# marekrams/tnac4o

Hardware: AMD Instinct MI355X
Metric: PEPS-contraction ms/sweep, chimera L=2048 chi=64 (boundary-MPS sweep _setup_rhoT) (lower is better)
Workload: dtype f64; 1 GPU; chimera L=2048 (Nx=Ny=16, Nc=8), synthetic couplings seed 20260004, beta=3, chi=64; one sweep = 16 rows of MPO absorb + compress_mps; one step = the sweeps of the 4 lattice rotations of one instance; parallelism=1 GPU: 4 lattice rotations of one instance interleaved on 4 HIP streams, mode=sweep

## Files before the change

tnac4o_amd/csrc/common.h:

```cpp
#pragma once
#include <hip/hip_runtime.h>
#include <stdint.h>
#include <stdio.h>
#include <stdlib.h>
#include <string.h>

namespace tn {

void set_error(const char* fmt, ...);
const char* get_error();

inline int hip_fail(hipError_t e, const char* what) {
    set_error("%s: %s", what, hipGetErrorString(e));
    return (int)e > 0 ? (int)e : 1;
}

#define TN_CHECK_ARG(cond, msg)                \
    do {                                       \
        if (!(cond)) {                         \
            tn::set_error("%s: %s", __func__, msg); \
            return -1;                         \
        }                                      \
    } while (0)

// ... 78 lines not shown
struct Mat {
    double* p;
    int64_t rs, cs;
};
static inline Mat mat(double* p, int64_t rs, int64_t cs) { return Mat{p, rs, cs}; }
static inline Mat sub(Mat a, int64_t i, int64_t j) { return Mat{a.p + i * a.rs + j * a.cs, a.rs, a.cs}; }
static inline Mat tr(Mat a) { return Mat{a.p, a.cs, a.rs}; }

int gemm(hipStream_t st, int64_t M, int64_t N, int64_t K, double alpha, const double* A, int64_t rsa, int64_t csa,
         const double* B, int64_t rsb, int64_t csb, double beta, double* C, int64_t rsc, int64_t csc,
         int64_t batch = 1, int64_t bsa = 0, int64_t bsb = 0, int64_t bsc = 0, double* ws = nullptr,
         int64_t ws_bytes = 0);
int64_t gemm_ws_bytes(int64_t M, int64_t N, int64_t K, int64_t batch);
struct GemmExtra {
    const int* pairs = nullptr;
    const int* skip = nullptr;
    int pw = 0, mapA = 0, mapB = 0, mapC = 0;
    int force_splitk = 0;
    bool raw_partials = false;
    int* splitk_used = nullptr;
};
int gemm_forced_split(int64_t K, int s, int64_t* kchunk);
int gemm_ex(hipStream_t st, int64_t M, int64_t N, int64_t K, double alpha, const double* A, int64_t rsa, int64_t csa,
            const double* B, int64_t rsb, int64_t csb, double beta, double* C, int64_t rsc, int64_t csc, int64_t batch,
            int64_t bsa, int64_t bsb, int64_t bsc, double* ws, int64_t ws_bytes, const GemmExtra* x);

static inline int gemm(hipStream_t st, int64_t M, int64_t N, int64_t K, double alpha, Mat A, Mat B, double beta, Mat C,
                       double* ws = nullptr, int64_t ws_bytes = 0) {
    return gemm(st, M, N, K, alpha, A.p, A.rs, A.cs, B.p, B.rs, B.cs, beta, C.p, C.rs, C.cs, 1, 0, 0, 0, ws, ws_bytes);
}
int gemm_prof_family(int64_t M, int64_t N, int64_t K, int64_t rsc, int64_t csc);

int rank_update(hipStream_t st, int64_t m, int64_t n, int b, const double* W, int64_t wrs, int64_t wcs, const double* X, int64_t xrs,
                int64_t xcs, double* C, int64_t rsc, int64_t csc, const int* active);
static inline int rank_update(hipStream_t st, int64_t m, int64_t n, int b, Mat W, Mat X, Mat C, const int* active = nullptr) {
    return rank_update(st, m, n, b, W.p, W.rs, W.cs, X.p, X.rs, X.cs, C.p, C.rs, C.cs, active);
}

struct FactorProducts {
    int64_t Z, I, J, K1, N, Mhi, Mlo;
    const double* P; int64_t pz, pi, pk;
    const double* X; int64_t xk, xj, xn;
    const double* W; int64_t wm, wq;
    double* Out; int64_t oz, ohi, olo, on;
};
bool factor_products_fits(int64_t Z, int64_t I, int64_t J, int64_t K1, int64_t N, int64_t M);
inline bool factor_products_on() { return env_flag_on("TN_FACTOR_FUSED"); }
int factor_products(hipStream_t st, const FactorProducts& f);

constexpr int NBMAX = 64;

int gram_partial(hipStream_t st, const double* X, int64_t vs, int64_t es, int64_t L, int nvec, int w, const int* pairs,
                 int ngroups, int nchunk, double* part);
int gram_nchunk(int64_t L);

int eig_small(hipStream_t st, const double* part, int nchunk, int nvec, int ngroups, int mode, int max_sweeps,
              double dead_thresh, double* out, int* dead, int* nrot, double* maxoff, double relevant2 = 0.0, int allow_fast = 1);

int rows_times_small(hipStream_t st, double* X, int64_t rs, int64_t cs, int64_t nrows, int b, const double* S);

struct SvdRoundsJob {
    double* X; int64_t pitch, L; int nvp, w;
    const int* pairs; int ng, nr, nchunk;
    double* part; int64_t part_bytes; double* Js; int* nrot; double* maxoff;
    double relevant2, last_tol; int inner_first, inner_later;
    double* norms;
};
int svd_rounds_fused(hipStream_t st, const SvdRoundsJob& j);
int small_t_times_vecs(hipStream_t st, const double* S, double* X, int64_t vs, int64_t es, int64_t L, int nvec, int w,
// ... 143 lines not shown
```

tnac4o_amd/csrc/qr.hip:

```cpp
#include <stdlib.h>

#include <algorithm>
#include <map>
#include <mutex>
#include <tuple>
#include <vector>

#include "common.h"
#include "devprim.h"

namespace tn {

__global__ __launch_bounds__(256) void copy_mat_kernel(const double* __restrict__ S, int64_t srs, int64_t scs,
                                                       double* __restrict__ D, int64_t drs, int64_t dcs, int64_t m,
                                                       int64_t n, int colfast) {
    const int64_t e = (int64_t)blockIdx.x * 256 + threadIdx.x;
    if (e >= m * n) return;
    const int64_t i = colfast ? e / n : e % m, j = colfast ? e % n : e / m;
    D[i * drs + j * dcs] = S[i * srs + j * scs];
}

int copy_mat(hipStream_t st, const double* S, int64_t srs, int64_t scs, double* D, int64_t drs, int64_t dcs, int64_t m,
             int64_t n) {
    if (m <= 0 || n <= 0) return 0;
// ... 588 lines not shown
    for (int e = tid; e < k * n; e += 256) {
        const int i = e / n, c = e % n;
        const double sg = (As[i * n + i] < 0.0) ? -1.0 : 1.0;
        R[(int64_t)i * rrs + (int64_t)c * rcs] = (c >= i) ? sg * As[i * n + c] * ds : 0.0;
    }
    if (Q)
        for (int e = tid; e < m * k; e += 256) {
            const int r = e / k, j = e % k;
            const double sg = (As[j * n + j] < 0.0) ? -1.0 : 1.0;
            Q[(int64_t)r * qrs + (int64_t)j * qcs] = sg * Qs[e];
        }
}

static bool dbg_on() { static const bool on = env_flag_set("TN_DEBUG"); return on; }
static void dbg_check(hipStream_t st, const double* p, int64_t rs, int64_t cs, int64_t m, int64_t n, const char* what, int panel, int it) {
    if (!dbg_on()) return;
    std::vector<double> h((size_t)(m * n));
    (void)hipStreamSynchronize(st);
    for (int64_t i = 0; i < m; ++i)
        for (int64_t j = 0; j < n; ++j) (void)hipMemcpy(&h[i * n + j], p + i * rs + j * cs, 8, hipMemcpyDeviceToHost);
    double mx = 0, mn = 1e300; int bad = 0;
    for (double v : h) { if (!(v == v) || v > 1e300 || v < -1e300) ++bad; else { double a = v < 0 ? -v : v; if (a > mx) mx = a; if (a < mn) mn = a; } }
    fprintf(stderr, "[tn_qr dbg] panel %d it %d %-10s %lldx%lld nonfinite=%d max=%.3e min|.|=%.3e\n", panel, it, what, (long long)m, (long long)n, bad, mx, mn);
}

constexpr int QR_NBO_MAX = 256;
struct QrWs {
    double *Y, *Wq, *W, *UT, *UTq;
    double *G, *Tblk, *Zo, *Zo2, *tmpT;
    double *T, *X, *part, *Js, *Uinv, *Z, *Tri, *gemm_ws, *cn;
    int* dead;
    int* pairs;
    char* piv;
    int64_t gemm_ws_bytes;
    void* panel_ws;
    int64_t panel_bytes;
    void* cq_state = nullptr;
};

static int64_t qr_layout(int64_t m, int64_t n, int nb, char* base, QrWs* w) {
    const int64_t k = m < n ? m : n, P = cdiv(k, nb);
    WsCarve ws{base};
    double* Y = ws.take<double>(m * k * 8);
    double* Wq = ws.take<double>(m * k * 8);
    double* Wp = ws.take<double>(m * nb * 8);
    double* UT = ws.take<double>((int64_t)nb * nb * 8);
    double* UTq = ws.take<double>((int64_t)nb * nb * 8);
    double* T = ws.take<double>(P * nb * nb * 8);
    double* X = ws.take<double>((int64_t)nb * (n > k ? n : k) * 8);
    double* part = ws.take<double>((int64_t)64 * nb * nb * 8);
    double* Js = ws.take<double>((int64_t)nb * nb * 8);
    double* Uinv = ws.take<double>((int64_t)nb * nb * 8);
    double* Z = ws.take<double>(P * nb * nb * 8);
    double* Tri = ws.take<double>(P * nb * nb * 8);
    int* dead = ws.take<int>(nb * 4);
    double* cn = ws.take<double>(2 * n * 8);
    int* pairs = ws.take<int>((int64_t)2 * nb * 4);
    char* piv = ws.take<char>(1024 + n * 4);
    int64_t gw = (int64_t)64 * nb * (n > k ? n : k) * 8;
    {
        const int64_t tiles = cdiv(QR_NBO_MAX, 128) * cdiv(n > k ? n : k, 128);
        const int64_t g2 = (512 + 2 * tiles) * 128 * 128 * 8;
        if (g2 > gw) gw = g2;
    }
    double* gws = ws.take<double>(gw + 256);
    const int64_t nblk_o = cdiv(k, QR_NBO_MAX / 2);
    double* Gm = ws.take<double>((int64_t)QR_NBO_MAX * QR_NBO_MAX * 8);
    double* Tblk = ws.take<double>(nblk_o * QR_NBO_MAX * QR_NBO_MAX * 8);
    double* Zb = ws.take<double>((int64_t)QR_NBO_MAX * (n > k ? n : k) * 8);
    double* Zb2 = ws.take<double>((int64_t)QR_NBO_MAX * (n > k ? n : k) * 8);
    double* tmpT = ws.take<double>((int64_t)QR_NBO_MAX * 64 * 8);
    if (w) { w->G = Gm; w->Tblk = Tblk; w->Zo = Zb; w->Zo2 = Zb2; w->tmpT = tmpT; }
    const int64_t pb = cholqr_ws_bytes(m, nb < 32 ? nb : 32);
    void* pw = ws.take(pb);
    if (w) { w->panel_ws = pw; w->panel_bytes = pb; }
    if (w) { w->Wq = Wq; w->W = Wp; w->UT = UT; w->UTq = UTq; }
    if (w) { w->Y = Y; w->T = T; w->X = X; w->part = part; w->Js = Js; w->Uinv = Uinv; w->Z = Z; w->Tri = Tri;
             w->dead = dead; w->gemm_ws = gws; w->gemm_ws_bytes = gw; w->cn = cn; w->pairs = pairs; w->piv = piv; }
    return ws.total();
}

int64_t qr_ws_bytes(int64_t m, int64_t n, int nb) { return qr_layout(m, n, nb, nullptr, nullptr); }
struct QrCall {
    hipStream_t st;
    double* A; int64_t rs, cs, m, n; double* Q; int64_t qrs, qcs; double* R; int64_t rrs, rcs;
    int nb; void* ws; int64_t ws_bytes; double rank_tol;
    int64_t* keff_host; double* dropped2_host; int frob_exit; int64_t* pivot_perm_host; double* nf_out2; int* nf_done; bool* input_intact;
};
struct QrState {
    QrWs w;
    bool pivot, reveal, rowmajor, ru_on, wform;
    int64_t yrs, ycs, wrs, wcs;
    Mat Am, Ym, Wqm;
    int fbase = 0;
    double scale2 = -1.0;
};
struct QrPanel {
    int p, b; int64_t j0, mp;
    Mat Ap, Yp, Wp, Wqp;
    double* Tp;
};
static QrPanel panel_at(const QrCall& c, const QrState& s, int p, int64_t kend) {
    QrPanel pn;
    pn.p = p, pn.j0 = (int64_t)p * c.nb, pn.mp = c.m - pn.j0;
    pn.b = (int)((kend - pn.j0 < c.nb) ? kend - pn.j0 : c.nb);
    pn.Ap = sub(s.Am, pn.j0, pn.j0), pn.Yp = sub(s.Ym, pn.j0, pn.j0), pn.Wqp = sub(s.Wqm, pn.j0, pn.j0);
    pn.Wp = s.wform ? pn.Wqp : mat(s.w.W, s.wrs, s.wcs);
    pn.Tp = s.w.T + (int64_t)p * c.nb * c.nb;
    return pn;
}
#define QR_LAUNCH(c, kernel, grid, ...) \
// ... 155 lines not shown
        S->h.k_exit = j0 + b;
        S->h.stamp = p + 1;
        if (p == 0) { S->h.scale2 = fro2; S->h.dropped2 = 0.0; }
        S->h.active = 1;
        piv_post(mail, 1, j0 + b, stamp);
    }
}
__global__ __launch_bounds__(256) void swap_columns_dev_kernel(double* __restrict__ A, int64_t rs, int64_t cs, int64_t m, const PivState* __restrict__ S,
                                                               int* __restrict__ perm) {
    const int g = threadIdx.x >> 6;
    int src[16], dst[16];
#pragma unroll
    for (int i = 0; i < 16; ++i) { src[i] = S->src[g * 16 + i]; dst[i] = S->dst[g * 16 + i]; }
    const int active = S->h.active, ns = S->h.swap_n;
    if (active == 0 || ns <= 0 || ns > 64) return;
    if (blockIdx.x == gridDim.x - 1) {
        int old = 0;
        if ((int)threadIdx.x < ns) old = perm[S->src[threadIdx.x]];
        __syncthreads();
        if ((int)threadIdx.x < ns) perm[S->dst[threadIdx.x]] = old;
        return;
    }
    const int64_t r = (int64_t)blockIdx.x * 64 + (threadIdx.x & 63);
    const bool in = r < m;
    double* row = A + (in ? r : 0) * rs;
    double v[16];
#pragma unroll
    for (int i = 0; i < 16; ++i) { const int t = g * 16 + i; v[i] = (in && t < ns) ? row[(int64_t)src[i] * cs] : 0.0; }
    __syncthreads();
#pragma unroll
    for (int i = 0; i < 16; ++i) { const int t = g * 16 + i; if (in && t < ns) row[(int64_t)dst[i] * cs] = v[i]; }
}

constexpr int QMB = 128;
__global__ __launch_bounds__(256) void zero_above_panels_kernel(double* __restrict__ Y, int64_t rs, int64_t cs, int64_t k, int nb) {
    const int64_t J0 = (int64_t)blockIdx.y * QMB;
    const int bw = (int)((k - J0 < QMB) ? k - J0 : QMB);
    for (int e = blockIdx.x * 256 + threadIdx.x; e < bw * bw; e += gridDim.x * 256) {
        const int i = e / bw, j = e % bw;
        if (i / nb < j / nb) Y[(J0 + i) * rs + (J0 + j) * cs] = 0.0;
    }
}
__global__ __launch_bounds__(256) void apply_merged_T_kernel(const double* __restrict__ Z, int64_t nq, const double* __restrict__ G, int bw,
                                                             const double* __restrict__ T, int npan, double* __restrict__ X) {
    constexpr int NP = QMB / 32;
    __shared__ double xs[QMB][33];
    __shared__ double vs[32][33];
    __shared__ double gs[(NP - 1) * 32][QMB - 32 + 1];
    __shared__ double ts[NP][32][33];
    const int tid = threadIdx.x, lane = tid & 63, wave = tid >> 6;
    const int lr = lane & 15, lk = lane >> 4, ti = wave >> 1, tj = wave & 1;
    const int64_t c0 = (int64_t)blockIdx.x * 32;
    {
        double gv[12][3], tv[NP * 4];
#pragma unroll
        for (int u1 = 0; u1 < 12; ++u1)
#pragma unroll
            for (int u2 = 0; u2 < 3; ++u2) {
                const int i = (tid >> 5) + 8 * u1, j = (tid & 31) + 32 * u2;
                const int col = 32 * ((i >> 5) + 1) + j;
                gv[u1][u2] = (i < (npan - 1) * 32 && col < bw) ? G[(int64_t)i * bw + col] : 0.0;
            }
#pragma unroll
        for (int u = 0; u < NP * 4; ++u) {
            const int q = u >> 2, idx = (u & 3) * 256 + tid, i = idx >> 5, l = idx & 31;
            const int bq = (bw - 32 * q < 32) ? bw - 32 * q : 32;
// ... 72 lines not shown
        for (size_t i = 0; i < v.size() && i < rows; ++i) {
            auto& k = v[i].second;
            auto& st = tab[k];
            fprintf(stderr, "  %6lld %6lld  %d %d %d : %6ld  %8.2f  %8.2f  %7.1f\n", (long long)std::get<0>(k), (long long)std::get<1>(k), std::get<2>(k),
                    std::get<3>(k), std::get<4>(k), st.second, st.first, 1e3 * st.first / st.second, ranks[k] / st.second);
        }
    }
};
QrTrace g_qr_trace;
}
static int single_launch_done(const QrCall& c, int64_t k, bool* done) {
    if (c.keff_host) *c.keff_host = k;
    if (c.input_intact) *c.input_intact = true;
    *done = true;
    return 0;
}
static int tiny_exit(const QrCall& c, int64_t k, bool* done) {
    const bool tiny_on = env_flag_on("TN_QR_TINY");
    if (!(tiny_on && c.nb == 32 && c.pivot_perm_host == nullptr && c.m * c.n <= 4096 && k <= 32)) return 0;
    QR_LAUNCH(c, tiny_qr_kernel, dim3(1), (const double*)c.A, c.rs, c.cs, (int)c.m, (int)c.n, c.Q, c.qrs, c.qcs, c.R, c.rrs, c.rcs);
    return single_launch_done(c, k, done);
}
static int smallqr_exit(const QrCall& c, QrWs& w, int64_t k, bool* done) {
    if (!(c.nb == 32 && c.pivot_perm_host == nullptr && c.Q != nullptr && smallqr_fits(c.m, c.n))) return 0;
    const int rc = smallqr_factor(c.st, c.A, c.rs, c.cs, c.m, c.n, c.Q, c.qrs, c.qcs, c.R, c.rrs, c.rcs, c.nf_out2, w.gemm_ws, w.gemm_ws_bytes);
    if (rc) return rc == 1 ? 0 : rc;
    if (c.nf_done) *c.nf_done = c.nf_out2 ? 1 : 0;
    return single_launch_done(c, k, done);
}
struct PivDev {
    PivState* pst = nullptr; int* pperm = nullptr;
    const int* active = nullptr;
    PivMail* ring = nullptr; unsigned seq0 = 0;
    int begin(const QrCall& c, QrWs& w, int P) {
        pst = (PivState*)w.piv, pperm = (int*)(w.piv + 1024), active = &pst->h.active;
        ring = (PivMail*)pinned_host(4 * sizeof(PivMail), PIN_SHARED);
        if (!ring) { set_error("tn_qr: no page-locked memory for the pivoting verdicts"); return 1; }
        for (int i = 0; i < 4; ++i) __atomic_store_n(&ring[i].word, 0ull, __ATOMIC_RELAXED);
        thread_local unsigned piv_seq = 0;
        seq0 = piv_seq, piv_seq += (unsigned)P + 1u;
        QR_LAUNCH(c, pivot_init_kernel, dim3((unsigned)cdiv(std::max<int64_t>(c.n, 256), 256)), pst, pperm, (int)c.n);
        return 0;
    }
    int select(const QrCall& c, QrWs& w, const QrPanel& pn) {
        const int64_t ntr = c.n - pn.j0;
        QR_LAUNCH(c, colnorm2_kernel, dim3((unsigned)ntr), pn.Ap.p, c.rs, c.cs, pn.mp, ntr, w.cn);
        QR_LAUNCH(c, pivot_select_kernel, dim3((unsigned)cdiv(ntr, PIV_CPB)), (const double*)w.cn, (int)ntr, pn.b, (int)pn.j0, pn.p, c.rank_tol * c.rank_tol, pst,
                  &ring[pn.p & 3], seq0 + (unsigned)pn.p + 1u);
        QR_LAUNCH(c, swap_columns_dev_kernel, dim3((unsigned)cdiv(c.m, 64) + 1), c.A, c.rs, c.cs, c.m, (const PivState*)pst, pperm);
        return 0;
    }
    int verdict(const QrCall& c, int q, bool* stop, int64_t* k_exit) {
        const PivMail* h = &ring[q & 3];
        const unsigned want = seq0 + (unsigned)q + 1u;
        unsigned long long wd = __atomic_load_n(&h->word, __ATOMIC_ACQUIRE);
        for (long spins = 0; (unsigned)(wd >> 32) != want; ++spins) {
            if ((spins & 0xfffff) == 0xfffff && hipStreamQuery(c.st) != hipErrorNotReady) {
                wd = __atomic_load_n(&h->word, __ATOMIC_ACQUIRE);
                if ((unsigned)(wd >> 32) == want) break;
                set_error("tn_qr: the pivoting verdict of panel %d never arrived", q);
                return 1;
            }
            wd = __atomic_load_n(&h->word, __ATOMIC_ACQUIRE);
        }
        *stop = ((wd >> 31) & 1ull) == 0ull;
        if (*stop) *k_exit = (int64_t)(wd & 0x7fffffffull);
        return 0;
    }
    int finish(const QrCall& c, QrWs& w, int P, bool* stop, int64_t* k_exit) {
        int rc;
        if (P >= 1 && !*stop && (rc = verdict(c, P - 1, stop, k_exit))) return rc;
        int* hp = nullptr;
        if ((rc = read_back_staged(c.st, (void**)&hp, w.piv, 1024 + (size_t)c.n * 4, PIN_QR, "permutation"))) return rc;
        for (int64_t j = 0; j < c.n; ++j) c.pivot_perm_host[j] = hp[256 + j];
        if (((const PivState*)hp)->h.stamp < 0) {
            set_error("tn_qr: the device-side pivot selection of panel %d was not a valid set of columns (TN_PIVOT_DEVICE=0 selects on the host)", -((const PivState*)hp)->h.stamp - 1);
            return 1;
        }
        if (*stop && c.dropped2_host) *c.dropped2_host = ((const PivState*)hp)->h.dropped2;
        return 0;
    }
};
static int pivot_on_host(const QrCall& c, QrState& s, const QrPanel& pn, bool* stop, int64_t* k_exit) {
    const int64_t ntr = c.n - pn.j0;
    int rc;
    QR_LAUNCH(c, colnorm2_kernel, dim3((unsigned)ntr), pn.Ap.p, c.rs, c.cs, pn.mp, ntr, s.w.cn);
    double* hcn = nullptr;
    if ((rc = read_back_staged(c.st, (void**)&hcn, s.w.cn, (size_t)ntr * 8, PIN_QR, "norms"))) return rc;
    double fro2 = 0.0;
    for (int64_t j = 0; j < ntr; ++j) fro2 += hcn[j];
    if (pn.p == 0) s.scale2 = fro2;
    if (pn.p > 0 && fro2 <= c.rank_tol * c.rank_tol * s.scale2) {
        if (c.dropped2_host) *c.dropped2_host = fro2;
        *stop = true, *k_exit = pn.j0;
        return 0;
    }
    int pairs[64];
    select_pivots(hcn, ntr, pn.b, pn.j0, c.pivot_perm_host, pairs);
    SwapList sl = {};
    compose_swaps(pairs, pn.b, sl);
    if (sl.n > 0)
        TN_PROF_LAUNCH(c.st, PROF_QR_AUX, hipLaunchKernelGGL(swap_columns_kernel, dim3((unsigned)cdiv(c.m, 256)), dim3(256), 0, c.st, c.A, c.rs, c.cs, c.m, sl));
    TN_CHECK_LAUNCH("swap_columns_kernel");
    return 0;
// ... 7 lines not shown
}
static int panel_jacobi64(const QrCall& c, QrState& s, const QrPanel& pn) {
    hipStream_t st = c.st;
    QrWs& w = s.w;
    const Mat Yp = pn.Yp, Wp = pn.Wp, Wqp = pn.Wqp;
    const int64_t yrs = s.yrs, ycs = s.ycs, mp = pn.mp;
    int rc, b = pn.b, p = pn.p;
    if ((rc = copy_mat(st, pn.Ap.p, c.rs, c.cs, Yp.p, yrs, ycs, mp, b))) return rc;
    const int nchunk = gram_nchunk(mp);
    for (int it = 0; it < 5; ++it) {
        if ((rc = gram_partial(st, Yp.p, ycs, yrs, mp, b, b, nullptr, 1, nchunk, w.part))) return rc;
        const int mode = (it < 4) ? 0 : 1;
        if ((rc = eig_small(st, w.part, nchunk, b, 1, mode, 12, it == 0 ? 0.0 : 1e-26, w.Js, mode == 0 ? w.dead : nullptr, nullptr, nullptr))) return rc;
        dbg_check(st, w.Js, b, 1, b, b, "Js", p, it);
        if ((rc = rows_times_small(st, Yp.p, yrs, ycs, mp, b, w.Js))) return rc;
        dbg_check(st, Yp.p, yrs, ycs, mp < 64 ? mp : 64, b, "W", p, it);
        if (mode == 0)
            QR_LAUNCH(c, refill_dead_kernel, dim3((unsigned)cdiv(mp, 256)), Yp.p, yrs, ycs, mp, b, w.dead, (uint64_t)(0x9E3779B97F4A7C15ULL * (uint64_t)(p * 4 + it + 1)));
    }
    TN_PROF_LAUNCH(st, PROF_LU, hipLaunchKernelGGL((lu_reconstruct_kernel<64>), dim3(1), dim3(256), 0, st, Yp.p, yrs, ycs, b, w.Uinv, pn.Tp, w.UT, w.UTq,
                       Wp.p, s.wrs, s.wcs, Wqp.p));
    TN_CHECK_LAUNCH("lu_reconstruct_kernel");
    dbg_check_factors(c, s, pn);
    if (mp > b) {
        dim3 grid((unsigned)cdiv(mp - b, 256));
        prof_begin(st, PROF_ROWS_SMALL);
        hipLaunchKernelGGL((rows_times_small3_kernel<64>), grid, dim3(256), 0, st, sub(Yp, b, 0).p, yrs, ycs, mp - b, b,
                           w.Uinv, w.UT, w.UTq, sub(Wp, b, 0).p, s.wrs, s.wcs, sub(Wqp, b, 0).p);
        TN_CHECK_LAUNCH("rows_times_small3_kernel");
        prof_end(st, PROF_ROWS_SMALL, 6.0 * (mp - b) * b * b, 32.0 * (mp - b) * b);
    }
    return 0;
}
static int trailing_update(const QrCall& c, QrState& s, const QrPanel& pn, int64_t nc, const int* active) {
    QrWs& w = s.w;
    const Mat Ap = pn.Ap, Wp = pn.Wp, Xm = mat(w.X, nc, 1), Yt = tr(pn.Yp);
    int rc;
    if (!active) {
        if ((rc = gemm(c.st, pn.b, nc, pn.mp, 1.0, Yt, Ap, 0.0, Xm, w.gemm_ws, w.gemm_ws_bytes))) return rc;
        return s.ru_on ? rank_update(c.st, pn.mp, nc, pn.b, Wp, Xm, Ap) : gemm(c.st, pn.mp, nc, pn.b, -1.0, Wp, Xm, 1.0, Ap);
    }
    GemmExtra gx_active;
    gx_active.skip = active;
    if ((rc = gemm_ex(c.st, pn.b, nc, pn.mp, 1.0, Yt.p, Yt.rs, Yt.cs, Ap.p, Ap.rs, Ap.cs, 0.0, Xm.p, Xm.rs, Xm.cs, 1, 0, 0, 0, w.gemm_ws, w.gemm_ws_bytes, &gx_active)))
        return rc;
    return s.ru_on ? rank_update(c.st, pn.mp, nc, pn.b, Wp, Xm, Ap, active)
                   : gemm_ex(c.st, pn.mp, nc, pn.b, -1.0, Wp.p, Wp.rs, Wp.cs, Xm.p, Xm.rs, Xm.cs, 1.0, Ap.p, Ap.rs, Ap.cs, 1, 0, 0, 0, nullptr, 0, &gx_active);
}
static int reveal_check(const QrCall& c, QrState& s, const QrPanel& pn, bool* stop, int64_t* k_exit) {
    double* cn = s.w.cn;
    const int64_t n = c.n, j1 = pn.j0 + pn.b, nt = n - j1;
    int rc;
    QR_LAUNCH(c, colnorm2_kernel, dim3((unsigned)nt), sub(s.Am, j1, j1).p, c.rs, c.cs, c.m - j1, nt, cn + n);
    const size_t nread = (size_t)(s.scale2 < 0.0 ? n + nt : nt);
    double* hcn = nullptr;
    if ((rc = read_back_staged(c.st, (void**)&hcn, s.scale2 < 0.0 ? cn : cn + n, nread * 8, PIN_QR, "norms"))) return rc;
    const double* tr2 = hcn;
    if (s.scale2 < 0.0) {
        s.scale2 = 0.0;
        for (int64_t j = 0; j < n; ++j) s.scale2 = c.frob_exit ? s.scale2 + hcn[j] : std::max(s.scale2, hcn[j]);
        tr2 = hcn + n;
    }
    double left = 0.0;
    for (int64_t j = 0; j < nt; ++j) left = c.frob_exit ? left + tr2[j] : std::max(left, tr2[j]);
    if (!(left <= c.rank_tol * c.rank_tol * s.scale2)) return 0;
    double fro2 = 0.0;
    for (int64_t j = 0; c.dropped2_host && j < nt; ++j) fro2 += tr2[j];
    if (c.dropped2_host) *c.dropped2_host = fro2;
    *stop = true, *k_exit = j1;
    return 0;
}
static int accumulate_Q_blocks(const QrCall& c, QrState& s, int64_t k, int bwo, bool merged_T) {
    hipStream_t st = c.st;
    QrWs& w = s.w;
    const int nb = c.nb, nblk = (int)cdiv(k, bwo);
    const Mat Qm = mat(c.Q, c.qrs, c.qcs);
    int rc;
    if (merged_T) QR_LAUNCH(c, zero_above_panels_kernel, dim3(16, (unsigned)nblk), w.Y, s.yrs, s.ycs, k, nb);
    for (int bi = nblk - 1; bi >= 0; --bi) {
// ... 75 lines not shown
    if (c.dropped2_host) *c.dropped2_host = 0.0;
    TN_CHECK_ARG(nb == 32 || nb == 64, "nb must be 32 or 64");
    TN_CHECK_ARG(c.ws_bytes >= qr_ws_bytes(m, n, nb), "workspace too small");
    int64_t k = m < n ? m : n;
    int rc;
    bool done = false, stop = false;
    if ((rc = tiny_exit(c, k, &done)) || done) return rc;
    QrState s;
    QrWs& w = s.w;
    qr_layout(m, n, nb, (char*)c.ws, &w);
    if ((rc = smallqr_exit(c, w, k, &done)) || done) return rc;
    int P = (int)cdiv(k, nb);
    const bool truncating = c.rank_tol > 0.0 && c.keff_host != nullptr;
    s.pivot = c.pivot_perm_host != nullptr && truncating && nb == 32;
    for (int64_t j = 0; c.pivot_perm_host && j < n; ++j) c.pivot_perm_host[j] = j;
    s.reveal = !s.pivot && truncating && P > 2 && nb == 32;
    if (s.reveal) QR_LAUNCH(c, colnorm2_kernel, dim3((unsigned)n), c.A, c.rs, c.cs, m, n, w.cn);
    s.rowmajor = (c.cs == 1 && c.rs != 1);
    s.yrs = s.rowmajor ? k : 1, s.ycs = s.rowmajor ? 1 : m, s.wrs = s.rowmajor ? nb : 1, s.wcs = s.rowmajor ? 1 : m;
    s.Am = mat(c.A, c.rs, c.cs), s.Ym = mat(w.Y, s.yrs, s.ycs), s.Wqm = mat(w.Wq, s.yrs, s.ycs);
    s.wform = (nb == 32);
    if (nb == 32 && (rc = cholqr_begin(c.st, w.panel_ws, &w.cq_state))) return rc;
    s.ru_on = nb == 32 && env_flag_on("TN_QR_RANK_UPDATE");
    {
        const int v_nbo = env_int("TN_QR_NBO", 256), nbo = (v_nbo == 128 || v_nbo == 256) ? v_nbo : 0;
        if (nbo > 0 && nb == 32 && !truncating && k >= 2 * nbo && m >= 4 * nbo) {
            if (c.keff_host) *c.keff_host = k;
            return qr_two_level(c, s, nbo);
        }
    }
    const bool piv_dev = s.pivot && env_flag_on("TN_PIVOT_DEVICE") && n <= PIV_MAXN;
    PivDev piv;
    if (piv_dev && (rc = piv.begin(c, w, P))) return rc;
    int64_t k_exit = k;
    for (int p = 0; p < P && !stop; ++p) {
        const QrPanel pn = panel_at(c, s, p, k);
        if (piv_dev) {
            if (p >= 1 && (rc = piv.verdict(c, p - 1, &stop, &k_exit))) return rc;
            if (!stop && (rc = piv.select(c, w, pn))) return rc;
        } else if (s.pivot && (rc = pivot_on_host(c, s, pn, &stop, &k_exit))) return rc;
        if (stop) break;
        if ((rc = s.wform ? panel_fused(c, s, pn, piv.active) : panel_jacobi64(c, s, pn))) return rc;
        if (s.wform) dbg_check_factors(c, s, pn);
        if ((rc = trailing_update(c, s, pn, n - pn.j0, piv.active))) return rc;
        if (s.reveal && (p & 1) == 1 && p + 1 < P && (rc = reveal_check(c, s, pn, &stop, &k_exit))) return rc;
    }
    if (piv_dev && (rc = piv.finish(c, w, P, &stop, &k_exit))) return rc;
    if (stop) k = k_exit, P = (int)(k / nb);
    if (c.keff_host) *c.keff_host = k;
    if (nb == 64) QR_LAUNCH(c, (diag_qr_kernel<64>), dim3(P), c.A, c.rs, c.cs, nb, k, w.Z, w.Tri, (int*)nullptr);
    else if ((rc = triangularise_diag(c, s, k, P))) return rc;
    dbg_check(c.st, w.Z, nb, 1, (int64_t)P * nb, nb, "Z", -1, 0);
    dbg_check(c.st, w.Tri, nb, 1, (int64_t)P * nb, nb, "Tri", -1, 0);
    const int64_t jf = (int64_t)(P - 1) * nb;
    const int fold_b = (nb == 32 && P >= 1 && m * k <= 256 * 512) ? (int)(k - jf) : 0;
    if ((rc = assemble_R_init_Q(c, s, k, QrFold{s.wform ? w.Wq : w.Y, s.wform ? w.Y : w.Wq, s.yrs, s.ycs, jf, fold_b}))) return rc;
    const bool merged_q = s.wform && c.Q != nullptr && P >= 2 && fold_b == 0 && env_flag_on("TN_QR_MERGED_Q");
    return merged_q ? accumulate_Q_blocks(c, s, k, QMB, true) : accumulate_Q_panels(c, s, k, P, fold_b);
}
static int qr_factor_traced(const QrCall& c) {
    if (c.nf_done) *c.nf_done = 0;
    if (!g_qr_trace.on) return qr_factor_impl(c);
    thread_local hipEvent_t e0 = nullptr, e1 = nullptr;
    if (!e0) { (void)hipEventCreate(&e0); (void)hipEventCreate(&e1); }
    (void)hipEventRecord(e0, c.st);
    const int rc = qr_factor_impl(c);
    (void)hipEventRecord(e1, c.st);
    (void)hipEventSynchronize(e1);
    float ms = 0.f;
    (void)hipEventElapsedTime(&ms, e0, e1);
    std::lock_guard<std::mutex> lk(g_qr_trace.mu);
    const bool truncating = c.rank_tol > 0.0 && c.keff_host;
    const auto key = std::make_tuple(c.m, c.n, c.Q ? 1 : 0, truncating ? 1 : 0, c.pivot_perm_host ? 1 : 0);
    auto& ss = g_qr_trace.tab[key];
    ss.first += ms, ss.second += 1;
    const double kr = c.keff_host ? (double)*c.keff_host : (double)(c.m < c.n ? c.m : c.n);
    g_qr_trace.ranks[key] += kr;
// ... 26 lines not shown
```

tnac4o_amd/csrc/rank_update.hip:

```cpp
#include "common.h"

namespace tn {

namespace {

typedef double d4 __attribute__((ext_vector_type(4)));
typedef double d2 __attribute__((ext_vector_type(2)));
typedef d2 d2u __attribute__((aligned(8)));

struct RankP {
    const double* A;
    const double* B;
    double* C;
    int M, N, K;
    int64_t rsa, csa, rsb, csb, rsc, csc;
    int tiles_n;
    const int* active;
};

template <int KG, bool WIDE>
__device__ __forceinline__ void rank_update_piece(const RankP& g, const int r0, const int c0, const int lr, const int lk, const int act) {
    double a[2][KG], b[2][KG], cv[2][2][4];
#pragma unroll
    for (int i = 0; i < 2; ++i) {
        const double* pa = g.A + (int64_t)min(r0 + i * 16 + lr, g.M - 1) * g.rsa;
#pragma unroll
        for (int kk = 0; kk < KG; ++kk) a[i][kk] = pa[(int64_t)min(kk * 4 + lk, g.K - 1) * g.csa];
    }
    if constexpr (WIDE) {
        const double* pb = g.B + (c0 + 2 * lr);
#pragma unroll
        for (int kk = 0; kk < KG; ++kk) {
            const d2 v = *(const d2u*)(pb + (int64_t)min(kk * 4 + lk, g.K - 1) * g.rsb);
            b[0][kk] = v.x; b[1][kk] = v.y;
        }
#pragma unroll
        for (int i = 0; i < 2; ++i)
#pragma unroll
            for (int r = 0; r < 4; ++r) {
                const d2 v = *(const d2u*)(g.C + (int64_t)(r0 + i * 16 + lk + 4 * r) * g.rsc + (c0 + 2 * lr));
                cv[i][0][r] = v.x; cv[i][1][r] = v.y;
            }
    } else {
#pragma unroll
        for (int j = 0; j < 2; ++j) {
            const double* pb = g.B + (int64_t)min(c0 + 2 * lr + j, g.N - 1) * g.csb;
#pragma unroll
            for (int kk = 0; kk < KG; ++kk) b[j][kk] = pb[(int64_t)min(kk * 4 + lk, g.K - 1) * g.rsb];
        }
#pragma unroll
        for (int i = 0; i < 2; ++i)
#pragma unroll
            for (int j = 0; j < 2; ++j)
#pragma unroll
                for (int r = 0; r < 4; ++r)
                    cv[i][j][r] = g.C[(int64_t)min(r0 + i * 16 + lk + 4 * r, g.M - 1) * g.rsc + (int64_t)min(c0 + 2 * lr + j, g.N - 1) * g.csc];
    }
    __builtin_amdgcn_sched_barrier(0);

    d4 acc[2][2];
#pragma unroll
    for (int i = 0; i < 2; ++i)
#pragma unroll
        for (int j = 0; j < 2; ++j) acc[i][j] = d4{0.0, 0.0, 0.0, 0.0};
#pragma unroll
    for (int kk = 0; kk < KG; ++kk) {
        const bool kin = kk * 4 + lk < g.K;
#pragma unroll
        for (int i = 0; i < 2; ++i)
#pragma unroll
            for (int j = 0; j < 2; ++j)
                acc[i][j] = __builtin_amdgcn_mfma_f64_16x16x4f64(kin ? a[i][kk] : 0.0, kin ? b[j][kk] : 0.0, acc[i][j], 0, 0, 0);
    }
#pragma unroll
    for (int i = 0; i < 2; ++i)
#pragma unroll
        for (int j = 0; j < 2; ++j)
#pragma unroll
            for (int r = 0; r < 4; ++r) cv[i][j][r] -= acc[i][j][r];
    __builtin_amdgcn_sched_barrier(0);

    if (!act) return;
    if constexpr (WIDE) {
#pragma unroll
        for (int i = 0; i < 2; ++i)
#pragma unroll
            for (int r = 0; r < 4; ++r)
                *(d2u*)(g.C + (int64_t)(r0 + i * 16 + lk + 4 * r) * g.rsc + (c0 + 2 * lr)) = d2{cv[i][0][r], cv[i][1][r]};
    } else {
#pragma unroll
        for (int i = 0; i < 2; ++i)
#pragma unroll
            for (int j = 0; j < 2; ++j)
#pragma unroll
                for (int r = 0; r < 4; ++r) {
                    const int row = r0 + i * 16 + lk + 4 * r, col = c0 + 2 * lr + j;
                    if (row < g.M && col < g.N) g.C[(int64_t)row * g.rsc + (int64_t)col * g.csc] = cv[i][j][r];
                }
    }
}

template <int KG, bool FLAG>
__global__ __launch_bounds__(256, 2) void rank_update_kernel(RankP g) {
    const int tid = threadIdx.x, lane = tid & 63, wave = __builtin_amdgcn_readfirstlane(tid >> 6);
    const int wm = wave >> 1, wn = wave & 1, lr = lane & 15, lk = lane >> 4;
    int bid = blockIdx.x;
    {
        const int nwg = gridDim.x, q = nwg / 8, r = nwg % 8, xcd = bid % 8, loc = bid / 8;
        bid = (xcd < r ? xcd * (q + 1) : r * (q + 1) + (xcd - r) * q) + loc;
    }
    const int r0 = (bid / g.tiles_n) * 64 + wm * 32, c0 = (bid % g.tiles_n) * 64 + wn * 32;
    if (r0 >= g.M || c0 >= g.N) return;
    const int act = FLAG ? *g.active : 1;
    if (r0 + 32 <= g.M && c0 + 32 <= g.N && g.csc == 1 && g.csb == 1) rank_update_piece<KG, true>(g, r0, c0, lr, lk, act);
    else rank_update_piece<KG, false>(g, r0, c0, lr, lk, act);
}

}

int rank_update(hipStream_t st, int64_t m, int64_t n, int b, const double* W, int64_t wrs, int64_t wcs, const double* X, int64_t xrs,
                int64_t xcs, double* C, int64_t rsc, int64_t csc, const int* active) {
    if (m <= 0 || n <= 0) return 0;
    TN_CHECK_ARG(b >= 1 && b <= 32, "the rank must be between 1 and 32");
    TN_CHECK_ARG(cdiv(m, 64) * cdiv(n, 64) < ((int64_t)1 << 31), "too many tiles");
    RankP g;
    g.C = C; g.K = b; g.active = active;
    if (rsc == 1 && csc != 1) {
        g.A = X; g.rsa = xcs; g.csa = xrs; g.B = W; g.rsb = wcs; g.csb = wrs; g.M = (int)n; g.N = (int)m; g.rsc = csc; g.csc = rsc;
    } else {
        g.A = W; g.rsa = wrs; g.csa = wcs; g.B = X; g.rsb = xrs; g.csb = xcs; g.M = (int)m; g.N = (int)n; g.rsc = rsc; g.csc = csc;
    }
    g.tiles_n = (int)cdiv(g.N, 64);
    const dim3 grid((unsigned)(cdiv(g.M, 64) * g.tiles_n));
    const int fam = gemm_prof_family(m, n, b, rsc, csc);
    prof_begin(st, fam);
    if (b <= 16 && active) hipLaunchKernelGGL((rank_update_kernel<4, true>), grid, dim3(256), 0, st, g);
    else if (b <= 16) hipLaunchKernelGGL((rank_update_kernel<4, false>), grid, dim3(256), 0, st, g);
    else if (active) hipLaunchKernelGGL((rank_update_kernel<8, true>), grid, dim3(256), 0, st, g);
    else hipLaunchKernelGGL((rank_update_kernel<8, false>), grid, dim3(256), 0, st, g);
    TN_CHECK_LAUNCH("rank_update_kernel");
    prof_end(st, fam, 2.0 * m * n * b, 8.0 * ((double)m * b + (double)b * n + 2.0 * m * n));
    return 0;
}

}
```

Baseline: 355.1 ms/sweep.

## Fuse pivot column-norm partial sums into QR trailing rank update

The rank-update kernel of the pivoted blocked QR now writes per-32-row partial squared column norms of the updated trailing matrix into a workspace. The next panel's pivot selection reduces these partials with a small kernel instead of rereading the whole trailing panel with colnorm2. A finish-time path recomputes the norms for the dropped tail when the QR stops early. This saves a full read of the trailing matrix per panel, at the cost of extra shuffles and stores in the rank update and a new workspace buffer.

```diff
diff --git a/tnac4o_amd/csrc/common.h b/tnac4o_amd/csrc/common.h
--- a/tnac4o_amd/csrc/common.h
+++ b/tnac4o_amd/csrc/common.h
@@ -134,9 +134,10 @@
 int gemm_prof_family(int64_t M, int64_t N, int64_t K, int64_t rsc, int64_t csc);
 
 int rank_update(hipStream_t st, int64_t m, int64_t n, int b, const double* W, int64_t wrs, int64_t wcs, const double* X, int64_t xrs,
-                int64_t xcs, double* C, int64_t rsc, int64_t csc, const int* active);
-static inline int rank_update(hipStream_t st, int64_t m, int64_t n, int b, Mat W, Mat X, Mat C, const int* active = nullptr) {
-    return rank_update(st, m, n, b, W.p, W.rs, W.cs, X.p, X.rs, X.cs, C.p, C.rs, C.cs, active);
+                int64_t xcs, double* C, int64_t rsc, int64_t csc, const int* active, double* norms_part);
+static inline int rank_update(hipStream_t st, int64_t m, int64_t n, int b, Mat W, Mat X, Mat C, const int* active = nullptr,
+                              double* norms_part = nullptr) {
+    return rank_update(st, m, n, b, W.p, W.rs, W.cs, X.p, X.rs, X.cs, C.p, C.rs, C.cs, active, norms_part);
 }
 
 struct FactorProducts {
diff --git a/tnac4o_amd/csrc/qr.hip b/tnac4o_amd/csrc/qr.hip
--- a/tnac4o_amd/csrc/qr.hip
+++ b/tnac4o_amd/csrc/qr.hip
@@ -644,6 +644,7 @@
     int* dead;
     int* pairs;
     char* piv;
+    double* nrm;
     int64_t gemm_ws_bytes;
     void* panel_ws;
     int64_t panel_bytes;
@@ -669,6 +670,7 @@
     double* cn = ws.take<double>(2 * n * 8);
     int* pairs = ws.take<int>((int64_t)2 * nb * 4);
     char* piv = ws.take<char>(1024 + n * 4);
+    double* nrm = ws.take<double>(nb == 32 ? cdiv(m, 32) * n * 8 : 0);
     int64_t gw = (int64_t)64 * nb * (n > k ? n : k) * 8;
     {
         const int64_t tiles = cdiv(QR_NBO_MAX, 128) * cdiv(n > k ? n : k, 128);
@@ -688,7 +690,7 @@
     if (w) { w->panel_ws = pw; w->panel_bytes = pb; }
     if (w) { w->Wq = Wq; w->W = Wp; w->UT = UT; w->UTq = UTq; }
     if (w) { w->Y = Y; w->T = T; w->X = X; w->part = part; w->Js = Js; w->Uinv = Uinv; w->Z = Z; w->Tri = Tri;
-             w->dead = dead; w->gemm_ws = gws; w->gemm_ws_bytes = gw; w->cn = cn; w->pairs = pairs; w->piv = piv; }
+             w->dead = dead; w->gemm_ws = gws; w->gemm_ws_bytes = gw; w->cn = cn; w->pairs = pairs; w->piv = piv; w->nrm = nrm; }
     return ws.total();
 }
 
@@ -910,6 +912,44 @@
     for (int i = 0; i < 16; ++i) { const int t = g * 16 + i; if (in && t < ns) row[(int64_t)dst[i] * cs] = v[i]; }
 }
 
+__global__ __launch_bounds__(256) void norm_reduce_kernel(const double* __restrict__ part, int64_t pld, int npc, int ntr, double* __restrict__ cn,
+                                                          const int* __restrict__ active) {
+    __shared__ double red[16][17];
+    if (*active == 0) return;
+    const int c = threadIdx.x & 15, q = threadIdx.x >> 4, j = blockIdx.x * 16 + c;
+    const double* pj = part + 32 + (j < ntr ? j : ntr - 1);
+    double s = 0.0;
+    for (int pc = 1 + q; pc < npc; pc += 128) {
+        double v[8];
+#pragma unroll
+        for (int u = 0; u < 8; ++u) v[u] = (pc + 16 * u < npc) ? pj[(int64_t)(pc + 16 * u) * pld] : 0.0;
+#pragma unroll
+        for (int u = 0; u < 8; ++u) s += v[u];
+    }
+    red[q][c] = s;
+    __syncthreads();
+    if (q == 0 && j < ntr) {
+        double t[16];
+#pragma unroll
+        for (int u = 0; u < 16; ++u) t[u] = red[u][c];
+#pragma unroll
+        for (int w = 1; w < 16; w <<= 1)
+#pragma unroll
+            for (int u = 0; u < 16; u += 2 * w) t[u] += t[u + w];
+        cn[j] = t[0];
+    }
+}
+__global__ __launch_bounds__(256) void dropped2_kernel(const double* __restrict__ cn, int ntr, PivState* S) {
+    __shared__ double red[256];
+    const int tid = threadIdx.x;
+    double part = 0.0;
+    for (int j = tid; j < ntr; j += 256) part += cn[j];
+    red[tid] = part;
+    __syncthreads();
+    for (int k = 128; k > 0; k >>= 1) { if (tid < k) red[tid] += red[tid + k]; __syncthreads(); }
+    if (tid == 0 && S->h.stamp > 0) S->h.dropped2 = red[0];
+}
+
 constexpr int QMB = 128;
 __global__ __launch_bounds__(256) void zero_above_panels_kernel(double* __restrict__ Y, int64_t rs, int64_t cs, int64_t k, int nb) {
     const int64_t J0 = (int64_t)blockIdx.y * QMB;
@@ -1048,6 +1088,7 @@
     PivState* pst = nullptr; int* pperm = nullptr;
     const int* active = nullptr;
     PivMail* ring = nullptr; unsigned seq0 = 0;
+    double* part = nullptr;
     int begin(const QrCall& c, QrWs& w, int P) {
         pst = (PivState*)w.piv, pperm = (int*)(w.piv + 1024), active = &pst->h.active;
         ring = (PivMail*)pinned_host(4 * sizeof(PivMail), PIN_SHARED);
@@ -1060,7 +1101,16 @@
     }
     int select(const QrCall& c, QrWs& w, const QrPanel& pn) {
         const int64_t ntr = c.n - pn.j0;
-        QR_LAUNCH(c, colnorm2_kernel, dim3((unsigned)ntr), pn.Ap.p, c.rs, c.cs, pn.mp, ntr, w.cn);
+        prof_begin(c.st, PROF_QR_AUX);
+        if (part && pn.p > 0) {
+            const int64_t npc = cdiv(pn.mp + c.nb, 32);
+            hipLaunchKernelGGL(norm_reduce_kernel, dim3((unsigned)cdiv(ntr, 16)), dim3(256), 0, c.st, (const double*)part, ntr + c.nb, (int)npc, (int)ntr, w.cn, active);
+            prof_end(c.st, PROF_QR_AUX, 0.0, 8.0 * (double)(npc - 1) * ntr);
+        } else {
+            hipLaunchKernelGGL(colnorm2_kernel, dim3((unsigned)ntr), dim3(256), 0, c.st, (const double*)pn.Ap.p, c.rs, c.cs, pn.mp, ntr, w.cn);
+            prof_end(c.st, PROF_QR_AUX, 0.0, 8.0 * (double)pn.mp * ntr);
+        }
+        TN_CHECK_LAUNCH("norm launch of the pivot selection");
         QR_LAUNCH(c, pivot_select_kernel, dim3((unsigned)cdiv(ntr, PIV_CPB)), (const double*)w.cn, (int)ntr, pn.b, (int)pn.j0, pn.p, c.rank_tol * c.rank_tol, pst,
                   &ring[pn.p & 3], seq0 + (unsigned)pn.p + 1u);
         QR_LAUNCH(c, swap_columns_dev_kernel, dim3((unsigned)cdiv(c.m, 64) + 1), c.A, c.rs, c.cs, c.m, (const PivState*)pst, pperm);
@@ -1086,6 +1136,11 @@
     int finish(const QrCall& c, QrWs& w, int P, bool* stop, int64_t* k_exit) {
         int rc;
         if (P >= 1 && !*stop && (rc = verdict(c, P - 1, stop, k_exit))) return rc;
+        if (*stop && part) {
+            const int64_t ntr = c.n - *k_exit, mp = c.m - *k_exit;
+            QR_LAUNCH(c, colnorm2_kernel, dim3((unsigned)ntr), (const double*)(c.A + *k_exit * (c.rs + c.cs)), c.rs, c.cs, mp, ntr, w.cn);
+            QR_LAUNCH(c, dropped2_kernel, dim3(1), (const double*)w.cn, (int)ntr, pst);
+        }
         int* hp = nullptr;
         if ((rc = read_back_staged(c.st, (void**)&hp, w.piv, 1024 + (size_t)c.n * 4, PIN_QR, "permutation"))) return rc;
         for (int64_t j = 0; j < c.n; ++j) c.pivot_perm_host[j] = hp[256 + j];
@@ -1159,7 +1214,7 @@
     }
     return 0;
 }
-static int trailing_update(const QrCall& c, QrState& s, const QrPanel& pn, int64_t nc, const int* active) {
+static int trailing_update(const QrCall& c, QrState& s, const QrPanel& pn, int64_t nc, const int* active, double* norms_part = nullptr) {
     QrWs& w = s.w;
     const Mat Ap = pn.Ap, Wp = pn.Wp, Xm = mat(w.X, nc, 1), Yt = tr(pn.Yp);
     int rc;
@@ -1171,7 +1226,7 @@
     gx_active.skip = active;
     if ((rc = gemm_ex(c.st, pn.b, nc, pn.mp, 1.0, Yt.p, Yt.rs, Yt.cs, Ap.p, Ap.rs, Ap.cs, 0.0, Xm.p, Xm.rs, Xm.cs, 1, 0, 0, 0, w.gemm_ws, w.gemm_ws_bytes, &gx_active)))
         return rc;
-    return s.ru_on ? rank_update(c.st, pn.mp, nc, pn.b, Wp, Xm, Ap, active)
+    return s.ru_on ? rank_update(c.st, pn.mp, nc, pn.b, Wp, Xm, Ap, active, norms_part)
                    : gemm_ex(c.st, pn.mp, nc, pn.b, -1.0, Wp.p, Wp.rs, Wp.cs, Xm.p, Xm.rs, Xm.cs, 1.0, Ap.p, Ap.rs, Ap.cs, 1, 0, 0, 0, nullptr, 0, &gx_active);
 }
 static int reveal_check(const QrCall& c, QrState& s, const QrPanel& pn, bool* stop, int64_t* k_exit) {
@@ -1313,6 +1368,7 @@
     const bool piv_dev = s.pivot && env_flag_on("TN_PIVOT_DEVICE") && n <= PIV_MAXN;
     PivDev piv;
     if (piv_dev && (rc = piv.begin(c, w, P))) return rc;
+    if (piv_dev && s.ru_on && env_flag_on("TN_QR_FUSED_NORMS")) piv.part = w.nrm;
     int64_t k_exit = k;
     for (int p = 0; p < P && !stop; ++p) {
         const QrPanel pn = panel_at(c, s, p, k);
@@ -1323,7 +1379,7 @@
         if (stop) break;
         if ((rc = s.wform ? panel_fused(c, s, pn, piv.active) : panel_jacobi64(c, s, pn))) return rc;
         if (s.wform) dbg_check_factors(c, s, pn);
-        if ((rc = trailing_update(c, s, pn, n - pn.j0, piv.active))) return rc;
+        if ((rc = trailing_update(c, s, pn, n - pn.j0, piv.active, p + 1 < P ? piv.part : nullptr))) return rc;
         if (s.reveal && (p & 1) == 1 && p + 1 < P && (rc = reveal_check(c, s, pn, &stop, &k_exit))) return rc;
     }
     if (piv_dev && (rc = piv.finish(c, w, P, &stop, &k_exit))) return rc;
diff --git a/tnac4o_amd/csrc/rank_update.hip b/tnac4o_amd/csrc/rank_update.hip
--- a/tnac4o_amd/csrc/rank_update.hip
+++ b/tnac4o_amd/csrc/rank_update.hip
@@ -16,9 +16,78 @@
     int64_t rsa, csa, rsb, csb, rsc, csc;
     int tiles_n;
     const int* active;
+    double* part;
+    int64_t pld;
+    int sum_n;
 };
 
-template <int KG, bool WIDE>
+template <int CTRL>
+__device__ __forceinline__ double ru_dpp(double v) {
+    int lo = __double2loint(v), hi = __double2hiint(v);
+    lo = __builtin_amdgcn_mov_dpp(lo, CTRL, 0xf, 0xf, true);
+    hi = __builtin_amdgcn_mov_dpp(hi, CTRL, 0xf, 0xf, true);
+    return __hiloint2double(hi, lo);
+}
+__device__ __forceinline__ double row16_sum(double s) {
+    s += ru_dpp<0xB1>(s);
+    s += ru_dpp<0x4E>(s);
+    s += ru_dpp<0x141>(s);
+    s += ru_dpp<0x140>(s);
+    return s;
+}
+
+template <bool WIDE>
+__device__ __forceinline__ void rank_update_norms(const RankP& g, const int r0, const int c0, const int lr, const int lk, const double (&cv)[2][2][4]) {
+    if (g.sum_n) {
+        const int pc = c0 >> 5;
+        if (pc == 0) return;
+        const bool in0 = WIDE || c0 + 2 * lr < g.N, in1 = WIDE || c0 + 2 * lr + 1 < g.N;
+        double s[2][4];
+#pragma unroll
+        for (int i = 0; i < 2; ++i)
+#pragma unroll
+            for (int r = 0; r < 4; ++r) {
+                const double x0 = in0 ? cv[i][0][r] : 0.0, x1 = in1 ? cv[i][1][r] : 0.0;
+                s[i][r] = row16_sum(__builtin_fma(x1, x1, x0 * x0));
+            }
+        if (lr != 0) return;
+        double* out = g.part + (int64_t)pc * g.pld;
+#pragma unroll
+        for (int i = 0; i < 2; ++i)
+#pragma unroll
+            for (int r = 0; r < 4; ++r) {
+                const int row = r0 + i * 16 + lk + 4 * r;
+                if (WIDE || row < g.M) out[row] = s[i][r];
+            }
+    } else {
+        const int pc = r0 >> 5;
+        if (pc == 0) return;
+        double t[2];
+#pragma unroll
+        for (int j = 0; j < 2; ++j) {
+            double a = 0.0;
+#pragma unroll
+            for (int i = 0; i < 2; ++i)
+#pragma unroll
+                for (int r = 0; r < 4; ++r) {
+                    const double x = (WIDE || r0 + i * 16 + lk + 4 * r < g.M) ? cv[i][j][r] : 0.0;
+                    a = __builtin_fma(x, x, a);
+                }
+            a += __shfl_xor(a, 16, 64);
+            a += __shfl_xor(a, 32, 64);
+            t[j] = a;
+        }
+        if (lk != 0) return;
+        double* out = g.part + (int64_t)pc * g.pld + (c0 + 2 * lr);
+        if constexpr (WIDE) *(d2u*)out = d2{t[0], t[1]};
+        else {
+            if (c0 + 2 * lr < g.N) out[0] = t[0];
+            if (c0 + 2 * lr + 1 < g.N) out[1] = t[1];
+        }
+    }
+}
+
+template <int KG, bool WIDE, bool NORMS>
 __device__ __forceinline__ void rank_update_piece(const RankP& g, const int r0, const int c0, const int lr, const int lk, const int act) {
     double a[2][KG], b[2][KG], cv[2][2][4];
 #pragma unroll
@@ -81,6 +150,7 @@
     __builtin_amdgcn_sched_barrier(0);
 
     if (!act) return;
+    if constexpr (NORMS) rank_update_norms<WIDE>(g, r0, c0, lr, lk, cv);
     if constexpr (WIDE) {
 #pragma unroll
         for (int i = 0; i < 2; ++i)
@@ -100,7 +170,7 @@
     }
 }
 
-template <int KG, bool FLAG>
+template <int KG, bool FLAG, bool NORMS>
 __global__ __launch_bounds__(256, 2) void rank_update_kernel(RankP g) {
     const int tid = threadIdx.x, lane = tid & 63, wave = __builtin_amdgcn_readfirstlane(tid >> 6);
     const int wm = wave >> 1, wn = wave & 1, lr = lane & 15, lk = lane >> 4;
@@ -112,34 +182,40 @@
     const int r0 = (bid / g.tiles_n) * 64 + wm * 32, c0 = (bid % g.tiles_n) * 64 + wn * 32;
     if (r0 >= g.M || c0 >= g.N) return;
     const int act = FLAG ? *g.active : 1;
-    if (r0 + 32 <= g.M && c0 + 32 <= g.N && g.csc == 1 && g.csb == 1) rank_update_piece<KG, true>(g, r0, c0, lr, lk, act);
-    else rank_update_piece<KG, false>(g, r0, c0, lr, lk, act);
-}
-
+    if (r0 + 32 <= g.M && c0 + 32 <= g.N && g.csc == 1 && g.csb == 1) rank_update_piece<KG, true, NORMS>(g, r0, c0, lr, lk, act);
+    else rank_update_piece<KG, false, NORMS>(g, r0, c0, lr, lk, act);
+}
+
+}
+
+template <bool NORMS>
+static void rank_update_launch(hipStream_t st, const dim3 grid, const RankP& g) {
+    if (g.K <= 16 && g.active) hipLaunchKernelGGL((rank_update_kernel<4, true, NORMS>), grid, dim3(256), 0, st, g);
+    else if (g.K <= 16) hipLaunchKernelGGL((rank_update_kernel<4, false, NORMS>), grid, dim3(256), 0, st, g);
+    else if (g.active) hipLaunchKernelGGL((rank_update_kernel<8, true, NORMS>), grid, dim3(256), 0, st, g);
+    else hipLaunchKernelGGL((rank_update_kernel<8, false, NORMS>), grid, dim3(256), 0, st, g);
 }
 
 int rank_update(hipStream_t st, int64_t m, int64_t n, int b, const double* W, int64_t wrs, int64_t wcs, const double* X, int64_t xrs,
-                int64_t xcs, double* C, int64_t rsc, int64_t csc, const int* active) {
+                int64_t xcs, double* C, int64_t rsc, int64_t csc, const int* active, double* norms_part) {
     if (m <= 0 || n <= 0) return 0;
     TN_CHECK_ARG(b >= 1 && b <= 32, "the rank must be between 1 and 32");
     TN_CHECK_ARG(cdiv(m, 64) * cdiv(n, 64) < ((int64_t)1 << 31), "too many tiles");
     RankP g;
-    g.C = C; g.K = b; g.active = active;
+    g.C = C; g.K = b; g.active = active; g.part = norms_part; g.pld = n;
     if (rsc == 1 && csc != 1) {
-        g.A = X; g.rsa = xcs; g.csa = xrs; g.B = W; g.rsb = wcs; g.csb = wrs; g.M = (int)n; g.N = (int)m; g.rsc = csc; g.csc = rsc;
-    } else {
-        g.A = W; g.rsa = wrs; g.csa = wcs; g.B = X; g.rsb = xrs; g.csb = xcs; g.M = (int)m; g.N = (int)n; g.rsc = rsc; g.csc = csc;
+        g.A = X; g.rsa = xcs; g.csa = xrs; g.B = W; g.rsb = wcs; g.csb = wrs; g.M = (int)n; g.N = (int)m; g.rsc = csc; g.csc = rsc; g.sum_n = 1;
+    } else {
+        g.A = W; g.rsa = wrs; g.csa = wcs; g.B = X; g.rsb = xrs; g.csb = xcs; g.M = (int)m; g.N = (int)n; g.rsc = rsc; g.csc = csc; g.sum_n = 0;
     }
     g.tiles_n = (int)cdiv(g.N, 64);
     const dim3 grid((unsigned)(cdiv(g.M, 64) * g.tiles_n));
     const int fam = gemm_prof_family(m, n, b, rsc, csc);
     prof_begin(st, fam);
-    if (b <= 16 && active) hipLaunchKernelGGL((rank_update_kernel<4, true>), grid, dim3(256), 0, st, g);
-    else if (b <= 16) hipLaunchKernelGGL((rank_update_kernel<4, false>), grid, dim3(256), 0, st, g);
-    else if (active) hipLaunchKernelGGL((rank_update_kernel<8, true>), grid, dim3(256), 0, st, g);
-    else hipLaunchKernelGGL((rank_update_kernel<8, false>), grid, dim3(256), 0, st, g);
+    if (norms_part) rank_update_launch<true>(st, grid, g);
+    else rank_update_launch<false>(st, grid, g);
     TN_CHECK_LAUNCH("rank_update_kernel");
-    prof_end(st, fam, 2.0 * m * n * b, 8.0 * ((double)m * b + (double)b * n + 2.0 * m * n));
+    prof_end(st, fam, 2.0 * m * n * b, 8.0 * ((double)m * b + (double)b * n + 2.0 * m * n + (norms_part ? (double)(cdiv(m, 32) - 1) * n : 0.0)));
     return 0;
 }
 
```

After: 356.8 ms/sweep. Within noise of the previous version (+0.5%).
